# TuringLang/AdvancedVI.jl

Measured on AMD Instinct MI355X. Metric: ELBO-grad-estimates/sec, higher is better.
Workload: dtype f32

## Files before the change

advancedvi.jl_amd/csrc/fr_planes.h:

```cpp
#pragma once
#include "device_common.h"

namespace mivi {

typedef float f32x16 __attribute__((ext_vector_type(16)));
typedef float f32x4 __attribute__((ext_vector_type(4)));
typedef _Float16 f16x8 __attribute__((ext_vector_type(8)));
typedef _Float16 f16x2 __attribute__((ext_vector_type(2)));
typedef unsigned u32x4v __attribute__((ext_vector_type(4)));

constexpr int kFrag = 512;
constexpr int kSplitProducts = 3;
constexpr float kEpsScale = 2048.f;
constexpr float kEpsInv = 1.f / 2048.f;

#define FB_GLDS16(gptr, lptr, off)                                                                         \
  __builtin_amdgcn_global_load_lds((const __attribute__((address_space(1))) void *)(gptr),                 \
                                   (__attribute__((address_space(3))) void *)(lptr), 16, off, 0)

template <int N>
__device__ __forceinline__ void fb_wait_vm() {
  __builtin_amdgcn_s_waitcnt((N & 15) | (7 << 4) | (15 << 8) | ((N >> 4) << 14));
  asm volatile("" ::: "memory");
}
__device__ __forceinline__ void fb_barrier() {
  __builtin_amdgcn_s_waitcnt(0xc07f);
  asm volatile("s_barrier" ::: "memory");
}

__device__ __forceinline__ void fb_scale_of(float amax, float &s, float &inv) {
  unsigned eb = (__builtin_bit_cast(unsigned, amax) >> 23) & 0xffu;
  eb = eb < 25u ? 25u : (eb > 254u ? 254u : eb);
  s = __builtin_bit_cast(float, (267u - eb) << 23);
  inv = __builtin_bit_cast(float, (eb - 13u) << 23);
}

__device__ __forceinline__ void fb_split2(const float *x, u32x4v &uh, u32x4v &ul) {
#pragma unroll
  for (int p = 0; p < 4; ++p) {
    const float a = x[2 * p], b = x[2 * p + 1];
    const _Float16 ah = (_Float16)a, bh = (_Float16)b;
    const float ra = a - (float)ah, rb = b - (float)bh;
    const f16x2 hh = {ah, bh}, ll = {(_Float16)ra, (_Float16)rb};
    uh[p] = __builtin_bit_cast(unsigned, hh);
    ul[p] = __builtin_bit_cast(unsigned, ll);
  }
}
__device__ __forceinline__ float fb_unsplit2(const u32x4v &uh, const u32x4v &ul, int e) {
  const unsigned wh = uh[e >> 1], wl = ul[e >> 1];
  const f16x2 hh = __builtin_bit_cast(f16x2, wh), ll = __builtin_bit_cast(f16x2, wl);
  return (float)hh[e & 1] + (float)ll[e & 1];
}
__device__ __forceinline__ float fb_unsplit2_word(unsigned wh, unsigned wl, int odd) {
  const f16x2 hh = __builtin_bit_cast(f16x2, wh), ll = __builtin_bit_cast(f16x2, wl);
  return (float)hh[odd] + (float)ll[odd];
}
__device__ __forceinline__ void fb_store_frag(unsigned *dst, const float *x) {
  u32x4v uh, ul;
  fb_split2(x, uh, ul);
  store16_wt(dst, uh);
  store16_wt(dst + 256, ul);
}

constexpr int kStageW = 16 * 256;

template <int WJ>
struct FbFrags {
  u32x4v A[2][2], B[WJ][2];
};
__device__ __forceinline__ f32x16 fb_mma(const u32x4v &a, const u32x4v &b, const f32x16 &c) {
  return __builtin_amdgcn_mfma_f32_32x32x16_f16(__builtin_bit_cast(f16x8, a), __builtin_bit_cast(f16x8, b), c, 0, 0, 0);
}
template <int WJ>
__device__ __forceinline__ void fb_group(const FbFrags<WJ> &F, f32x16 (&acc)[2][WJ]) {
  constexpr int PA[3] = {1, 0, 0}, PB[3] = {0, 1, 0};
#pragma unroll
  for (int p = 0; p < 3; ++p)
#pragma unroll
    for (int i = 0; i < 2; ++i)
#pragma unroll
      for (int j = 0; j < WJ; ++j) acc[i][j] = fb_mma(F.A[i][PA[p]], F.B[j][PB[p]], acc[i][j]);
}

template <int OFF>
__device__ __forceinline__ void fb_group_read_asm(f32x16 &acc0, f32x16 &acc1, const FbFrags<1> &Fc, FbFrags<1> &Fn, unsigned ab, unsigned bb) {
  static_assert(OFF >= 0 && OFF + 3072 < 65536, "ds_read_b128 offset field");
  asm volatile(
      "v_mfma_f32_32x32x16_f16 %[c0], %[a0l], %[bh], %[c0]\n\t"
      "ds_read_b128 %[n0h], %[ab] offset:%[o0]\n\t"
      "ds_read_b128 %[n0l], %[ab] offset:%[o1]\n\t"
      "v_mfma_f32_32x32x16_f16 %[c1], %[a1l], %[bh], %[c1]\n\t"
      "ds_read_b128 %[n1h], %[ab] offset:%[o2]\n\t"
      "ds_read_b128 %[n1l], %[ab] offset:%[o3]\n\t"
      "v_mfma_f32_32x32x16_f16 %[c0], %[a0h], %[bl], %[c0]\n\t"
      "ds_read_b128 %[nbh], %[bb] offset:%[o0]\n\t"
      "v_mfma_f32_32x32x16_f16 %[c1], %[a1h], %[bl], %[c1]\n\t"
      "ds_read_b128 %[nbl], %[bb] offset:%[o1]\n\t"
      "v_mfma_f32_32x32x16_f16 %[c0], %[a0h], %[bh], %[c0]\n\t"
      "v_mfma_f32_32x32x16_f16 %[c1], %[a1h], %[bh], %[c1]\n\t"
      "s_waitcnt lgkmcnt(0)"
      : [c0] "+v"(acc0), [c1] "+v"(acc1), [n0h] "=&v"(Fn.A[0][0]), [n0l] "=&v"(Fn.A[0][1]), [n1h] "=&v"(Fn.A[1][0]), [n1l] "=&v"(Fn.A[1][1]),
        [nbh] "=&v"(Fn.B[0][0]), [nbl] "=&v"(Fn.B[0][1])
      : [a0h] "v"(Fc.A[0][0]), [a0l] "v"(Fc.A[0][1]), [a1h] "v"(Fc.A[1][0]), [a1l] "v"(Fc.A[1][1]), [bh] "v"(Fc.B[0][0]), [bl] "v"(Fc.B[0][1]),
        [ab] "v"(ab), [bb] "v"(bb), [o0] "n"(OFF), [o1] "n"(OFF + 1024), [o2] "n"(OFF + 2048), [o3] "n"(OFF + 3072)
      : "memory");
}

template <int WJ>
__device__ __forceinline__ void fb_read_frags(const unsigned *lds, int slot, int wm, int wn, int lane, FbFrags<WJ> &F) {
  const unsigned *cur = lds + slot * kStageW + 4 * lane;
#pragma unroll
  for (int i = 0; i < 2; ++i)
#pragma unroll
    for (int p = 0; p < 2; ++p) F.A[i][p] = *(const u32x4v *)(cur + ((2 * wm + i) * 2 + p) * 256);
#pragma unroll
  for (int j = 0; j < WJ; ++j)
#pragma unroll
    for (int p = 0; p < 2; ++p) F.B[j][p] = *(const u32x4v *)(cur + (8 + (WJ * wn + j) * 2 + p) * 256);
}

}
```

advancedvi.jl_amd/csrc/kernels_fullrank_batch.hip:

```cpp
#include <algorithm>
#include <cstdlib>
#include <type_traits>
#include <cstdio>
#include <vector>

#include "device_common.h"
#include "fr_elem.h"
#include "fr_planes.h"

#ifndef FB_VK
#define FB_VK 0
#endif
#ifndef FB_WJ
#define FB_WJ 1
#endif

namespace mivi {

struct FbArgs {
  int d, M, L;
  int dT, MT;
  const float *params;
  const float *t_mean, *t_istd;
  unsigned *CA;
// ... 295 lines not shown
      FB_GLDS16(sp[f], dst, 0);
      FB_GLDS16(sp[f], dst, 1024);
      sp[f] += gd < gmax[f] ? kFrag : 0;
    }
    ++gd;
  };
  f32x16 acc[2][WJ];
#pragma unroll
  for (int i = 0; i < 2; ++i)
#pragma unroll
    for (int j = 0; j < WJ; ++j)
#pragma unroll
      for (int r = 0; r < 16; ++r) acc[i][j][r] = 0.f;
  const int r32[2] = {R0 + 2 * wm, R0 + 2 * wm + 1};
  const int Gw = (kDG || kSU) ? G : 2 * r32[1] + 2;
  auto after_group = [&](auto S, int g) {
    if constexpr (kDG && (decltype(S)::value & 3) == 3) {
      if (((g + 1) & 7) == 0) {
#pragma unroll
        for (int j = 0; j < WJ; ++j) {
          const float f = tab[((g >> 3) << 7) + 32 * (WJ * wn + j) + l31];
#pragma unroll
          for (int i = 0; i < 2; ++i) {
#pragma unroll
            for (int r = 0; r < 16; ++r) acc[i][j][r] *= f;
          }
        }
        asm volatile("" ::: "memory");
      }
    }
  };
  auto compute = [&](auto S, int g, const FbFrags<WJ> &F) {
    if (!FB_KNOCKED(a, 2)) fb_group<WJ>(F, acc);
    fb_sched_interleave<WJ>();
    after_group(S, g);
  };
  const unsigned lds0 = (unsigned)(uintptr_t)lds + 16u * lane;
  const unsigned ab_lo = lds0 + (2 * wm) * 2 * 1024, bb_lo = lds0 + (8 + WJ * wn * 2) * 1024;
  const unsigned ab_hi = ab_lo + 4 * kStageW * 4, bb_hi = bb_lo + 4 * kStageW * 4;
  (void)ab_hi; (void)bb_hi;
  auto step = [&](auto S, auto VM, auto ISS, int g, const FbFrags<WJ> &Fc, FbFrags<WJ> &Fn) {
    constexpr int sl = decltype(S)::value;
    fb_wait_vm<kPW * decltype(VM)::value>();
    if (!FB_KNOCKED(a, 8)) fb_barrier();
#ifdef MIVI_SB
    __builtin_amdgcn_sched_barrier(0);
#endif
    auto group_and_read = [&]() {
#ifndef MIVI_DEV
      if constexpr (WJ == 1) {
        constexpr int nx = (sl + 1) % NRP, off = (nx & 3) * kStageW * 4;
        fb_group_read_asm<off>(acc[0][0], acc[1][0], Fc, Fn, nx < 4 ? ab_lo : ab_hi, nx < 4 ? bb_lo : bb_hi);
        if constexpr (kDG && (sl & 3) == 3) {
          if (((g + 1) & 7) == 0) asm volatile("s_nop 15\n\ts_nop 7" : "+v"(acc[0][0]), "+v"(acc[1][0])::"memory");
        }
        after_group(S, g);
      } else
#endif
      {
        if (!FB_KNOCKED(a, 4)) fb_read_frags<WJ>(lds, (sl + 1) % NRP, wm, wn, lane, Fn);
        compute(S, g, Fc);
      }
    };
    if constexpr (decltype(ISS)::value) {
      if (!FB_KNOCKED(a, 1)) issue(sl);
      group_and_read();
    } else if (g < Gw) {
      group_and_read();
    }
  };
  FB_STAMP(a, 0);
  FB_NOTE(a, 4, G);
  load_tables();
  static_for<0, NRP>([&](auto S) { issue(decltype(S)::value); });
  fb_wait_vm<kPW * NRP>();
  stage_tables();
  fb_wait_vm<kPW * (NRP - 1)>();
  fb_barrier();
  FB_STAMP(a, 1);
  {
    FbFrags<WJ> F0, F1;
    fb_read_frags<WJ>(lds, 0, wm, wn, lane, F0);
    int g = 0;
    for (; g + NRP < G; g += NRP) {
      static_for<0, NRP>([&](auto S) {
        constexpr int sv = decltype(S)::value;
        if constexpr (sv % 2 == 0) step(S, std::integral_constant<int, NRP - 2>{}, FbT{}, g + sv, F0, F1);
        else step(S, std::integral_constant<int, NRP - 2>{}, FbT{}, g + sv, F1, F0);
      });
    }
    static_for<0, NRP - 1>([&](auto S) {
      constexpr int sv = decltype(S)::value;
      if constexpr (sv % 2 == 0) step(S, std::integral_constant<int, NRP - 2 - sv>{}, FbN{}, g + sv, F0, F1);
      else step(S, std::integral_constant<int, NRP - 2 - sv>{}, FbN{}, g + sv, F1, F0);
    });
    __builtin_amdgcn_s_waitcnt(0xc07f);
    if (g + NRP - 1 < Gw) compute(std::integral_constant<int, NRP - 1>{}, g + NRP - 1, F1);
  }
  f32x16 (&tot)[2][WJ] = acc;
  fb_barrier();
  FB_STAMP(a, 2);
  float *img = reinterpret_cast<float *>(lds) + w * (2 * WJ * kImgW);
  unsigned *WVl = a.WV + (size_t)ln * a.plane_stride;
  unsigned *RPl = a.RP + (size_t)ln * a.plane_stride;
  double *ellp = a.ell_part + (size_t)ln * a.ell_stride;
  const int ncb = a.M >> 5, nmg = a.M >> 4;
  const int ei4 = 4 * (lane & 7);
  float amax[2][4];
  float cmax[WJ][4];
#pragma unroll
  for (int i = 0; i < 2; ++i)
#pragma unroll
    for (int c = 0; c < 4; ++c) amax[i][c] = 0.f;
#pragma unroll
  for (int j = 0; j < WJ; ++j)
#pragma unroll
    for (int p = 0; p < 4; ++p) cmax[j][p] = 0.f;
#pragma unroll
  for (int i = 0; i < 2; ++i) {
    const int lr = 64 * wm + 32 * i;
    f32x4 mu = {0.f, 0.f, 0.f, 0.f}, tm = mu, tis = mu;
    const f32x4 zf = *(const f32x4 *)(vec + 384 + lr + ei4);
    if constexpr (!kDG && !kSU) {
      mu = *(const f32x4 *)(vec + lr + ei4);
      tm = *(const f32x4 *)(vec + 128 + lr + ei4);
      if constexpr (MODE == FB_DIAG) tis = *(const f32x4 *)(vec + 256 + lr + ei4);
    }
#pragma unroll
    for (int j = 0; j < WJ; ++j) {
      float *I = img + (i * WJ + j) * kImgW;
      const int cb32 = (col0 >> 5) + WJ * wn + j;
      const bool pad = 32 * r32[i] >= a.dT || 32 * cb32 >= a.MT;
#pragma unroll
      for (int q = 0; q < 4; ++q) {
        const f32x4 v = {tot[i][j][4 * q], tot[i][j][4 * q + 1], tot[i][j][4 * q + 2], tot[i][j][4 * q + 3]};
        *(f32x4 *)(I + l31 * LDC + 8 * q + 4 * h) = v;
      }
      if constexpr (kSU) {
        const float uf = vec[384 + lr + l31];
        const float wo = a.winv[(size_t)ln * (size_t)(a.M >> 7) * d + (size_t)cb * d + row0 + lr + l31];
#pragma unroll
        for (int g2 = 0; g2 < 2; ++g2) {
          const unsigned *src = WVl + ((size_t)r32[i] * nmg + 2 * cb32 + g2) * kFrag + 4 * lane;
          const u32x4v wh = *(const u32x4v *)src, wl = *(const u32x4v *)(src + 256);
#pragma unroll
          for (int e = 0; e < 8; ++e) {
            float *p = I + (16 * g2 + 8 * (e >> 2) + 4 * h + (e & 3)) * LDC + l31;
            const float x = __builtin_fmaf(*p, uf, fb_unsplit2(wh, wl, e) * wo);
            *p = x;
            amax[i][0] = fmaxf(amax[i][0], fabsf(x));
          }
        }
        continue;
      }
      double s = 0.0;
#pragma unroll
      for (int p = 0; p < 4; ++p) {
        const int en = 8 * p + (lane >> 3);
        const f32x4 v = *(const f32x4 *)(I + en * LDC + ei4) * zf;
        float ell = 0.f;
        f32x4 wv;
        if constexpr (MODE == FB_DIAG) {
          const f32x4 z = mu + v;
#pragma unroll
          for (int c = 0; c < 4; ++c) wv[c] = diag_target_elem(z[c], tm[c], tis[c], ell);
        } else if constexpr (kDR) {
          const f32x4 z = mu + v;
          wv = z - tm;
        } else {
          const unsigned *fr = RPl + ((size_t)cb32 * ng + 2 * r32[i] + (ei4 >> 4)) * kFrag + 4 * (en + 32 * ((ei4 >> 2) & 1)) + 2 * ((ei4 >> 3) & 1);
          const uint2 qh = *(const uint2 *)fr, ql = *(const uint2 *)(fr + 256);
          const float rs = rsv[32 * (WJ * wn + j) + en];
          const unsigned uh[2] = {qh.x, qh.y}, ul[2] = {ql.x, ql.y};
#pragma unroll
          for (int c = 0; c < 4; ++c) wv[c] = dense_target_elem(v[c], fb_unsplit2_word(uh[c >> 1], ul[c >> 1], c & 1) * rs, ell);
        }
        if (pad) { wv = f32x4{0.f, 0.f, 0.f, 0.f}; ell = 0.f; }
        *(f32x4 *)(I + en * LDC + ei4) = wv;
        if constexpr (kDR) {
          cmax[j][p] = fmaxf(cmax[j][p], fmaxf(fmaxf(fabsf(wv[0]), fabsf(wv[1])), fmaxf(fabsf(wv[2]), fabsf(wv[3]))));
        } else {
#pragma unroll
          for (int c = 0; c < 4; ++c) amax[i][c] = fmaxf(amax[i][c], fabsf(wv[c]));
          const double sv = (double)wave_sum_f32(ell);
          s = p ? s + sv : sv;
        }
      }
      if constexpr (!kDR) {
        if (lane == 0) ellp[(size_t)r32[i] * ncb + cb32] = s;
      }
    }
  }
  if constexpr (kDR) {
#pragma unroll
    for (int j = 0; j < WJ; ++j)
#pragma unroll
      for (int p = 0; p < 4; ++p) {
        const float m = fb_lane_max<7>(cmax[j][p]);
        if ((lane & 7) == 0) red[w * 64 + 32 * j + 8 * p + (lane >> 3)] = m;
      }
  } else if constexpr (kSU) {
#pragma unroll
    for (int i = 0; i < 2; ++i) {
      const float m = fb_lane_max<32>(amax[i][0]);
      if (lane < 32) red[w * 64 + 32 * i + lane] = m;
    }
  } else {
#pragma unroll
    for (int i = 0; i < 2; ++i)
#pragma unroll
      for (int c = 0; c < 4; ++c) {
        const float m = fb_lane_max<56>(amax[i][c]);
        if (lane < 8) red[w * 64 + 32 * i + ei4 + c] = m;
      }
  }
  fb_barrier();
  if constexpr (kDR) {
#pragma unroll
    for (int j = 0; j < WJ; ++j) {
      const int cb32 = (col0 >> 5) + WJ * wn + j;
      float s, inv;
      fb_scale_of(fmaxf(red[wn * 64 + 32 * j + l31], red[(NWN + wn) * 64 + 32 * j + l31]), s, inv);
      if (wm == 0 && lane < 32) a.rinv[(size_t)ln * (size_t)(d >> 7) * a.M + (size_t)rb * a.M + col0 + 32 * (WJ * wn + j) + lane] = inv;
#pragma unroll
      for (int i = 0; i < 2; ++i) {
        const float *I = img + (i * WJ + j) * kImgW;
#pragma unroll
        for (int g2 = 0; g2 < 2; ++g2) {
          const f32x4 x0 = *(const f32x4 *)(I + l31 * LDC + 16 * g2 + 4 * h) * s, x1 = *(const f32x4 *)(I + l31 * LDC + 16 * g2 + 8 + 4 * h) * s;
          const float x[8] = {x0[0], x0[1], x0[2], x0[3], x1[0], x1[1], x1[2], x1[3]};
          fb_store_frag(RPl + ((size_t)cb32 * ng + 2 * r32[i] + g2) * kFrag + 4 * lane, x);
        }
      }
    }
  } else {
#pragma unroll
    for (int i = 0; i < 2; ++i) {
      float mx = red[(wm * NWN) * 64 + 32 * i + l31];
#pragma unroll
      for (int x = 1; x < NWN; ++x) mx = fmaxf(mx, red[(wm * NWN + x) * 64 + 32 * i + l31]);
      float s, inv;
      fb_scale_of(mx, s, inv);
      if (wn == 0 && lane < 32) a.winv[(size_t)ln * (size_t)(a.M >> 7) * d + (size_t)cb * d + row0 + 64 * wm + 32 * i + lane] = inv;
#pragma unroll
      for (int j = 0; j < WJ; ++j) {
        const float *I = img + (i * WJ + j) * kImgW;
        const int cb32 = (col0 >> 5) + WJ * wn + j;
#pragma unroll
        for (int g2 = 0; g2 < 2; ++g2) {
          float x[8];
#pragma unroll
          for (int e = 0; e < 8; ++e) x[e] = I[(16 * g2 + 8 * (e >> 2) + 4 * h + (e & 3)) * LDC + l31] * s;
          fb_store_frag(WVl + ((size_t)r32[i] * nmg + 2 * cb32 + g2) * kFrag + 4 * lane, x);
        }
      }
    }
  }
  FB_STAMP(a, 3);
  if (!kDG && !kSU && (flags & 1) && wn == 0 && lane < 32) {
    const int nrb = d >> 5;
#pragma unroll
    for (int i = 0; i < 2; ++i) {
      const int r = 32 * r32[i] + lane;
      float lg, bad;
      logdet_block32(r < a.dT ? a.params[a.dT + (size_t)r * a.dT + r] : 1.f, lg, bad);
      if (lane == 0) {
        a.ld_part[r32[i]] = (double)lg;
        a.ld_part[nrb + r32[i]] = (double)bad;
      }
    }
  }
}

__device__ __forceinline__ void fb_value_block(const FbArgs &a, int l, double *red) {
  const int d = a.d;
  ValueIn vin{};
  vin.ell_const = a.ell_const;
  vin.ell_part = a.ell_part + (size_t)l * a.ell_stride;
  vin.n_ell_part = (d >> 5) * (a.M >> 5);
  vin.he_part = a.he_part + (size_t)l * a.he_stride;
  vin.n_he_part = (d >> 6) * (a.M >> 5);
  vin.ld_part = a.ld_part;
  vin.n_ld_part = d >> 5;
  OutArgs out{};
  const bool last = l == a.lane_last && a.value_last;
  out.value = last ? a.value_last : a.values + (size_t)l * a.value_stride;
  if (a.parts) {
    out.partials_mode = 1;
    out.partials = a.parts + (size_t)l * a.part_stride;
    out.scalars_off = (int64_t)d + (int64_t)(d >> 7) * ((d >> 7) + 1) / 2 * 16384;
  }
  out.ent_kind = a.ent_kind;
  out.M_total = a.M_total;
  out.M_local = a.MT;
  out.status = a.status;
  const float *pp = a.params;
  const int dT = a.dT;
  finalize_value_block<float, 256, false>(dT, vin, out, (int64_t)dT + (int64_t)dT * dT, [pp, dT](int i) { return pp[dT + (size_t)i * dT + i]; }, red);
}

template <int WJ, int NRV, int TABW, int WPE, bool PART = false>
__global__ __launch_bounds__(512 / WJ, WPE / WJ) void k_fb_vjp(FbArgs a) {
  static_assert(WJ == 1, "the transposing B reads are written for the 64 x 32 wave tiles");
  constexpr int LDC = 36, NF = WJ, kPW = 2 * WJ;
  constexpr int NR = NRV;
  constexpr int kBody = (NR * kStageW > 16 * kImgW / 2) ? NR * kStageW : 16 * kImgW / 2;
  __shared__ __attribute__((aligned(16))) unsigned lds[kBody + TABW];
  float *wf = reinterpret_cast<float *>(lds + kBody);
  const int tid = threadIdx.x, lane = tid & 63, l31 = lane & 31, h = lane >> 5;
  const int w = __builtin_amdgcn_readfirstlane(tid >> 6);
  const int wm = w / (4 / WJ), wn = w % (4 / WJ);
  if ((int)blockIdx.x < a.L) {
    if (tid < 256) fb_value_block(a, (int)blockIdx.x, reinterpret_cast<double *>(lds));
    return;
  }
  const __attribute__((address_space(4))) int *wp = (const __attribute__((address_space(4))) int *)a.work + 4 * ((int)blockIdx.x - a.L);
  const int ln = wp[0], rc = wp[1];
  const int rb = rc & 0xffff, cb = rc >> 16;
  const int d = a.d, M = a.M, nmg = M >> 4, dT = a.dT;
  const int row0 = rb * 128, col0 = cb * 128;
  const bool last = ln == a.lane_last && a.grad_last;
  float *grad = last ? a.grad_last : a.grads + (size_t)ln * a.grad_stride;
  const bool upper = a.write_upper || last;
  const int G = nmg;
  const int NB = M >> 7;
  const unsigned *sp[NF];
  unsigned btr;
  {
    const int G4 = lane >> 4, c16 = lane & 15;
    const int kgpar = G4 & 1, hq = G4 >> 1, hp = c16 & 1, half = (c16 >> 1) & 1, sl = 4 * hq + (c16 >> 2);
    btr = 16u * (unsigned)(8 * (2 * hp + kgpar) + ((sl & 7) ^ (4 * hp))) + 8u * (unsigned)half;
  }
#pragma unroll
  for (int f = 0; f < NF; ++f) {
    const int fs = NF * w + f, fr = fs & 3;
    if (fs < 4) {
      sp[f] = a.WV + (size_t)ln * a.plane_stride + ((size_t)((row0 >> 5) + fr) * nmg) * kFrag + 4 * lane;
    } else {
      const int m8 = lane >> 3, s8 = m8 >> 2, hp = (m8 >> 1) & 1, kgpar = m8 & 1, sl = 8 * s8 + ((lane & 7) ^ (4 * hp));
      sp[f] = a.epsP + (size_t)ln * a.plane_stride + ((size_t)((col0 >> 4) + 2 * fr + kgpar)) * kFrag + 4 * (sl + 32 * hp);
    }
  }
  int gi = 0;
  const int bstep_odd = (d >> 4) * kFrag - 64;
  constexpr int kMaxNBv = 16;
  float twi[kMaxNBv];
  auto load_table = [&]() {
    if (tid < 128) {
      const float *wi = a.winv + (size_t)ln * (size_t)NB * d + row0 + tid;
#pragma unroll
      for (int r = 0; r < kMaxNBv; ++r) twi[r] = wi[(size_t)(r < NB ? r : NB - 1) * d];
    }
    asm volatile("" ::: "memory");
  };
  auto build_table = [&]() {
    if (tid < 128) {
      float u = twi[0], grow = 1.f;
#pragma unroll
      for (int r = 1; r < kMaxNBv; ++r) {
        if (r < NB) {
          float ratio = u / twi[r];
          if (!(ratio <= 1099511627776.f)) ratio = 1099511627776.f;
          if (ratio > 1.f && grow * ratio > 1.2089258e24f) ratio = fmaxf(1.2089258e24f / grow, 1.f);
          if (ratio > 1.f) grow *= ratio;
          wf[(r - 1) * 128 + tid] = ratio;
          u = u / ratio;
        }
      }
      wf[(NB - 1) * 128 + tid] = u;
    }
  };
  auto issue = [&](int slot) {
#pragma unroll
    for (int f = 0; f < NF; ++f) {
      unsigned *dst = lds + slot * kStageW + (NF * w + f) * 512;
      if (!(FB_VK & 16)) {
        FB_GLDS16(sp[f], dst, 0);
        FB_GLDS16(sp[f], dst, 1024);
      }
      if (NF * w + f >= 4) sp[f] += (gi & 1) ? bstep_odd : 64;
      else sp[f] += kFrag;
    }
    ++gi;
  };
  auto read_frags = [&](int slot, FbFrags<WJ> &F) {
    if ((FB_VK & 64)) return;
    const unsigned *cur = lds + slot * kStageW + 4 * lane;
#pragma unroll
    for (int i = 0; i < 2; ++i)
#pragma unroll
      for (int p = 0; p < 2; ++p) F.A[i][p] = *(const u32x4v *)(cur + ((2 * wm + i) * 2 + p) * 256);
    const unsigned bb = (unsigned)(uintptr_t)(lds + slot * kStageW) + (8 + 2 * wn) * 1024 + btr;
    uint2 t0, t1, t2, t3;
    asm volatile("ds_read_b64_tr_b16 %0, %4\n\tds_read_b64_tr_b16 %1, %4 offset:512\n\tds_read_b64_tr_b16 %2, %4 offset:1024\n\t"
                 "ds_read_b64_tr_b16 %3, %4 offset:1536\n\ts_waitcnt lgkmcnt(0)"
                 : "=&v"(t0), "=&v"(t1), "=&v"(t2), "=&v"(t3) : "v"(bb) : "memory");
    F.B[0][0] = u32x4v{t0.x, t0.y, t1.x, t1.y};
    F.B[0][1] = u32x4v{t2.x, t2.y, t3.x, t3.y};
  };
  const int ri[2] = {(row0 >> 5) + 2 * wm, (row0 >> 5) + 2 * wm + 1};
  int cj[WJ];
#pragma unroll
  for (int j = 0; j < WJ; ++j) cj[j] = (col0 >> 5) + WJ * wn + j;
  const bool work = cj[0] <= ri[1];
  bool dg[2];
#pragma unroll
  for (int i = 0; i < 2; ++i) {
    dg[i] = false;
#pragma unroll
    for (int j = 0; j < WJ; ++j) dg[i] = dg[i] || ri[i] == cj[j];
  }
  f32x16 acc[2][WJ];
#pragma unroll
  for (int i = 0; i < 2; ++i)
#pragma unroll
    for (int j = 0; j < WJ; ++j)
#pragma unroll
      for (int r = 0; r < 16; ++r) acc[i][j][r] = 0.f;
  double rsd[2] = {0.0, 0.0};
  float rcur[2] = {0.f, 0.f};
  auto after_group = [&](auto S, int g, const FbFrags<WJ> &F) {
    if (__builtin_expect(dg[0] || dg[1], 0)) {
#pragma unroll
      for (int i = 0; i < 2; ++i)
        if (dg[i]) {
#pragma unroll
          for (int e = 0; e < 8; ++e) rcur[i] += fb_unsplit2(F.A[i][0], F.A[i][1], e);
        }
    }
    if constexpr (decltype(S)::value == 3 || decltype(S)::value == -1) {
      if (((g + 1) & 7) == 0 && g + 1 < G) {
        const float *wr = wf + ((g >> 3) << 7) + 64 * wm;
#pragma unroll
        for (int i = 0; i < 2; ++i) {
#pragma unroll
          for (int q = 0; q < 4; ++q) {
            const f32x4 f4 = *(const f32x4 *)(wr + 32 * i + 8 * q + 4 * h);
#pragma unroll
            for (int j = 0; j < WJ; ++j)
#pragma unroll
              for (int c = 0; c < 4; ++c) acc[i][j][4 * q + c] *= f4[c];
          }
          rsd[i] = (rsd[i] + (double)rcur[i]) * (double)wr[32 * i + l31];
          rcur[i] = 0.f;
        }
        asm volatile("" ::: "memory");
      }
    }
  };
  auto compute = [&](auto S, int g, const FbFrags<WJ> &F) {
    if (!(FB_VK & 32)) fb_group<WJ>(F, acc);
    after_group(S, g, F);
  };
  {
    FB_STAMP(a, 0);
    FB_NOTE(a, 4, G);
    load_table();
#pragma unroll
    for (int s0 = 0; s0 < NR - 1; ++s0) issue(s0);
    fb_wait_vm<kPW * (NR - 1)>();
    build_table();
    int slot = 0;
    for (int g = 0; g < G; ++g) {
      if (g == 1) FB_STAMP(a, 1);
      if (g + NR - 2 < G) fb_wait_vm<kPW * (NR - 2)>();
      else if (NR > 3 && g + 1 < G) fb_wait_vm<kPW>();
      else fb_wait_vm<0>();
      fb_barrier();
      if (g + NR - 1 < G) issue(slot == 0 ? NR - 1 : slot - 1);
      if (work) {
        FbFrags<WJ> F;
        read_frags(slot, F);
        compute(std::integral_constant<int, -1>{}, g, F);
      }
      slot = slot == NR - 1 ? 0 : slot + 1;
    }
  }
  fb_barrier();
  FB_STAMP(a, 2);
  if ((FB_VK & 128)) return;
  float *Cs = reinterpret_cast<float *>(lds) + w * kImgW;
  const float *wfin = wf + (NB - 1) * 128 + 64 * wm;
  const double invM = 1.0 / (double)a.M_total;
  const bool pow2M = (a.M_total & (a.M_total - 1)) == 0;
  const float invMe = (float)invM * kEpsInv;
  const double direct = direct_entropy_coeff(a.ent_kind);
  const int i4 = 4 * (lane & 7);
#pragma unroll
  for (int i = 0; i < 2; ++i) {
#pragma unroll
    for (int j = 0; j < WJ; ++j) {
      if (cj[j] > ri[i] || 32 * ri[i] >= dT) continue;
      const bool diag = ri[i] == cj[j];
      const int rbase = 32 * ri[i], cbase = 32 * cj[j];
#pragma unroll
      for (int q = 0; q < 4; ++q) {
        const f32x4 v = {acc[i][j][4 * q], acc[i][j][4 * q + 1], acc[i][j][4 * q + 2], acc[i][j][4 * q + 3]};
        *(f32x4 *)(Cs + l31 * LDC + 8 * q + 4 * h) = v;
      }
      const f32x4 ff = *(const f32x4 *)(wfin + 32 * i + i4);
#pragma unroll
      for (int p = 0; p < 4; ++p) {
        const int n = 8 * p + (lane >> 3);
        const int gi = rbase + i4, gj = cbase + n;
        float cjj = 1.f;
        if (diag && gj >= gi && gj < gi + 4) cjj = a.params[dT + (size_t)gj * dT + gj];
        const f32x4 v = *(const f32x4 *)(Cs + n * LDC + i4) * ff;
        f32x4 o;
        if constexpr (PART) {
          o = v * kEpsInv;
          if (diag) {
#pragma unroll
            for (int c = 0; c < 4; ++c) o[c] = gj > gi + c ? 0.f : o[c];
          }
          store16_wt(a.parts + (size_t)ln * a.part_stride + d + ((size_t)(rb * (rb + 1) / 2 + cb) << 14) + (size_t)(gj - col0) * 128 + (gi - row0), o);
          continue;
        }
        if (!diag && pow2M) {
          o = -v * invMe;
        } else {
#pragma unroll
          for (int c = 0; c < 4; ++c) o[c] = vjp_elem(v[c] * kEpsInv, gi + c, gj, pow2M, (float)invM, invM, direct, cjj);
        }
        store16_wt(grad + dT + (size_t)gj * dT + gi, o);
      }
      if (!PART && !diag && upper) {
        const f32x4 z4 = {0.f, 0.f, 0.f, 0.f};
#pragma unroll
        for (int p = 0; p < 4; ++p) {
          const int ii = 8 * p + (lane >> 3);
          store16_wt(grad + dT + (size_t)(rbase + ii) * dT + cbase + i4, z4);
        }
      }
      asm volatile("s_waitcnt lgkmcnt(0)" ::: "memory");
    }
    if (dg[i] && 32 * ri[i] < dT) {
      const double mine = (rsd[i] + (double)rcur[i]) * (double)wfin[32 * i + l31];
      const double sm = mine + __shfl_xor(mine, 32, 64);
      if constexpr (PART) {
        if (lane < 32) a.parts[(size_t)ln * a.part_stride + 32 * ri[i] + lane] = (float)sm;
      } else {
        if (lane < 32) grad[32 * ri[i] + lane] = dmu_elem(sm, invM);
      }
    }
  }
  FB_STAMP(a, 3);
}

__global__ __launch_bounds__(256) void k_fb_finalize_parts(FbArgs a) {
  __shared__ double red[4 * 4];
  const int d = a.d, l = blockIdx.y, j = blockIdx.x, tid = threadIdx.x;
  const float *P = a.parts + (size_t)l * a.part_stride;
  const bool last = l == a.lane_last && a.grad_last;
  float *grad = last ? a.grad_last : a.grads + (size_t)l * a.grad_stride;
  const bool upper = a.write_upper || last;
  const double invM = 1.0 / (double)a.M_total;
  const bool pow2M = (a.M_total & (a.M_total - 1)) == 0;
  const double direct = direct_entropy_coeff(a.ent_kind);
  if (j == d) {
    for (int i = tid; i < d; i += 256) grad[i] = dmu_elem((double)P[i], invM);
    double s_ld = 0.0, bad = 0.0;
    for (int i = tid; i < d; i += 256) {
      const double c = (double)a.params[d + (size_t)i * d + i];
      if (!(c > 0.0)) bad = 1.0;
      s_ld += log(c);
    }
    double v[2] = {s_ld, bad};
    block_sum_n<double, 256, 2>(v, red);
    if (tid == 0) {
      const int64_t so = (int64_t)d + (int64_t)(d >> 7) * ((d >> 7) + 1) / 2 * 16384;
      const double sum_ell = (double)P[so], s_he = (double)P[so + 1], Mt = (double)a.M_total;
      const double ent = (ent_is_closed(a.ent_kind) ? 0.5 * d * (1.0 + kLog2Pi) : s_he / Mt + 0.5 * d * kLog2Pi) + v[0];
      const double value = -(sum_ell / Mt + ent);
      float *vo = (l == a.lane_last && a.value_last) ? a.value_last : a.values + (size_t)l * a.value_stride;
      *vo = (float)value;
      int st = 0;
      if (!isfinite(value)) st |= 1;
      if (v[1] > 0.0) st |= 2;
      if (st && a.status) atomicOr(a.status, st);
    }
    return;
  }
  const int cb = j >> 7, lj = j & 127;
  const float cjj = a.params[d + (size_t)j * d + j];
  for (int i4 = 4 * tid; i4 < d; i4 += 1024) {
    f32x4 o = {0.f, 0.f, 0.f, 0.f};
    if (i4 + 3 >= j) {
      const int rb = i4 >> 7;
      const f32x4 v = *(const f32x4 *)(P + d + ((size_t)(rb * (rb + 1) / 2 + cb) << 14) + (size_t)lj * 128 + (i4 & 127));
#pragma unroll
      for (int c = 0; c < 4; ++c) o[c] = vjp_elem(v[c], i4 + c, j, pow2M, (float)invM, invM, direct, cjj);
    } else if (!upper) {
      continue;
    }
    *(f32x4 *)(grad + d + (size_t)j * d + i4) = o;
  }
}

namespace {
constexpr int kBM = 128, kBN = 128;
constexpr int kWJ = FB_WJ;
constexpr int kOwnCuTilesPerCU10 = 17;

void fb_upload(DevBuf &b, const void *src, size_t bytes) {
  if (b.bytes < bytes || !b.p) {
    if (b.p) (void)hipFree(b.p);
    (void)hipMalloc(&b.p, bytes);
    b.bytes = bytes;
  }
  (void)hipMemcpy(b.p, src, bytes, hipMemcpyHostToDevice);
}
}

static int fb_pad(int x) { return (x + 127) / 128 * 128; }
bool fb_shape_ok(const mivi_ctx *c, int M) {
  static const bool off = getenv("MIVI_BATCH_GEN3") && atoi(getenv("MIVI_BATCH_GEN3")) == 0;
  return !off && c->cfg.family == MIVI_FULLRANK && c->cfg.dtype == MIVI_F32 && c->cfg.d % 32 == 0 && M % 32 == 0 && c->cfg.d >= kBM &&
         c->cfg.d <= 2048 && M >= 128 && M <= 2048;
}
bool fb_whole_tiles(const mivi_ctx *c, int M) { return c->cfg.d % kBM == 0 && M % kBN == 0; }
size_t fb_plane_words(const mivi_ctx *c, int M) { return (size_t)fb_pad(c->cfg.d) * fb_pad(M) / 512 * kFrag; }
size_t fb_cplane_words(const mivi_ctx *c) { return (size_t)(fb_pad(c->cfg.d) / 32) * (fb_pad(c->cfg.d) / 16) * kFrag; }
size_t fb_part_len(const mivi_ctx *c) {
  const size_t d = (size_t)c->cfg.d, T = d / 128;
  return (d + T * (T + 1) / 2 * 16384 + 2 + 3) / 4 * 4;
}

const FbTab *fb_prepare(mivi_ctx *c, int M, int L) {
  FbTables &ft = c->fb;
  for (FbTab &t : ft.tab)
    if (t.L == L && t.M == M && t.prod.p && t.vjp.p) return &t;
  FbTab &t = ft.tab[ft.next_tab];
  ft.next_tab = (ft.next_tab + 1) & 3;
  invalidate_graph(c);
  (void)hipStreamSynchronize(c->stream);
  t.L = t.M = 0;
  const int d = fb_pad(c->cfg.d), nrb = d / kBM, ncb = fb_pad(M) / kBN;
  std::vector<std::vector<int4>> lists(8);
  int panel = 0;
  for (int l = 0; l < L; ++l)
    for (int cb = 0; cb < ncb; ++cb, ++panel)
      for (int rb = nrb - 1; rb >= 0; --rb) lists[panel % 8].push_back(make_int4(l, rb | (cb << 16), (l == 0 && cb == 0) ? 1 : 0, 0));
  while (true) {
    int a = 0, b = 0;
    for (int x = 1; x < 8; ++x) {
      if (lists[x].size() > lists[a].size()) a = x;
      if (lists[x].size() < lists[b].size()) b = x;
    }
    if (lists[a].size() <= lists[b].size() + 1) break;
    lists[b].push_back(lists[a].back());
    lists[a].pop_back();
  }
  for (auto &li : lists) std::stable_sort(li.begin(), li.end(), [](const int4 &p, const int4 &q) { return (p.y & 0xffff) > (q.y & 0xffff); });
  std::vector<int4> prod;
  size_t mx = 0;
  for (auto &li : lists) mx = std::max(mx, li.size());
  for (size_t i = 0; i < mx; ++i)
    for (int x = 0; x < 8; ++x)
      if (i < lists[x].size()) prod.push_back(lists[x][i]);
  std::vector<int4> flat;
  for (int l = 0; l < L; ++l)
    for (int rb = 0; rb < nrb; ++rb)
      for (int cb = 0; cb <= rb; ++cb) flat.push_back(make_int4(l, rb | (cb << 16), 0, 0));
  std::vector<int4> vjp;
  {
    const size_t n = flat.size();
    size_t pos = 0;
    std::vector<std::vector<int4>> lx(8);
    for (int x = 0; x < 8; ++x) {
      const size_t e = (n * (x + 1)) / 8;
      for (; pos < e; ++pos) lx[x].push_back(flat[pos]);
    }
    size_t m2 = 0;
    for (auto &li : lx) m2 = std::max(m2, li.size());
    for (size_t i = 0; i < m2; ++i)
      for (int x = 0; x < 8; ++x)
        if (i < lx[x].size()) vjp.push_back(lx[x][i]);
  }
  std::vector<int4> prod2;
  const size_t panel_bytes = (size_t)kBM * d * 4;
  constexpr int NG = 4, NC = 8 / NG;
  if (nrb % NG == 0 && (size_t)(nrb / NG) * panel_bytes <= (1u << 20)) {
    std::vector<std::vector<int4>> lp(8);
    int pn = 0;
    for (int l = 0; l < L; ++l)
      for (int cb = 0; cb < ncb; ++cb, ++pn)
        for (int rg = 0; rg < NG; ++rg)
          for (int r = 0; r < nrb / NG; ++r) lp[rg + NG * (pn % NC)].push_back(make_int4(l, (rg * (nrb / NG) + r) | (cb << 16), 0, 0));
    size_t m3 = 0;
    for (auto &li : lp) m3 = std::max(m3, li.size());
    for (size_t i = 0; i < m3; ++i)
      for (int x = 0; x < 8; ++x)
        if (i < lp[x].size()) prod2.push_back(lp[x][i]);
  } else {
    for (int l = 0; l < L; ++l)
      for (int cb = 0; cb < ncb; ++cb)
        for (int rb = 0; rb < nrb; ++rb) prod2.push_back(make_int4(l, rb | (cb << 16), 0, 0));
  }
  std::vector<int4> prod3;
  for (auto &li : lists) std::stable_sort(li.begin(), li.end(), [](const int4 &p, const int4 &q) { return (p.y & 0xffff) < (q.y & 0xffff); });
  for (size_t i = 0; i < mx; ++i)
    for (int x = 0; x < 8; ++x)
      if (i < lists[x].size()) prod3.push_back(lists[x][i]);
  fb_upload(t.prod, prod.data(), prod.size() * sizeof(int4));
  fb_upload(t.vjp, vjp.data(), vjp.size() * sizeof(int4));
  fb_upload(t.prod2, prod2.data(), prod2.size() * sizeof(int4));
  fb_upload(t.prod3, prod3.data(), prod3.size() * sizeof(int4));
  if (!t.prod.p || !t.vjp.p || !t.prod2.p || !t.prod3.p) return nullptr;
  t.n_prod2 = (int)prod2.size();
  t.n_prod = (int)prod.size();
  t.n_vjp = (int)vjp.size();
  t.L = L;
  t.M = M;
  return &t;
}

static FbArgs fb_args(mivi_ctx *c, const void *params, int M_true) {
  FbTables &t = c->fb;
  const int d = fb_pad(c->cfg.d), M = fb_pad(M_true);
  FbArgs a{};
  a.d = d; a.M = M;
  a.dT = c->cfg.d; a.MT = M_true;
  a.params = (const float *)params;
  a.t_mean = (const float *)c->t_mean.p;
  a.t_istd = (const float *)c->t_istd.p;
  a.CA = (unsigned *)t.CA.p;
  a.cscale = (float *)t.cscale.p;
  a.pscale = (float *)t.pscale.p;
  a.tscale = (float *)t.tscale.p;
  a.winv = (float *)t.winv.p;
  a.rinv = (float *)t.rinv.p;
  a.epsP = (unsigned *)t.epsP.p;
  a.WV = (unsigned *)t.WV.p;
  a.t_prec = (const float *)c->t_prec.p; a.dP = c->dP;
  a.PA = (unsigned *)t.PA.p;
  a.RP = (unsigned *)t.RP.p;
  a.Tinv = (const float *)t.Tinv.p;
  a.TA = (unsigned *)t.TA.p;
  a.plane_stride = (long long)fb_plane_words(c, M);
  a.ell_part = (double *)t.ell.p; a.ell_stride = (long long)(d / 32) * (M / 32);
  a.he_part = (double *)t.he.p; a.he_stride = (long long)(d / 64) * (M / 32);
  a.ld_part = (double *)t.ld.p;
  a.ent_kind = c->cfg.entropy; a.M_total = c->M_total;
  a.status = (int *)c->status.p;
  a.ell_const = c->t_const;
  return a;
}

void fb_launch_eps(mivi_ctx *c, const FbStep &s, bool with_cplanes, hipStream_t stream) {
  const int d = fb_pad(c->cfg.d), M = fb_pad(s.M), L = s.L;
  FbArgs a = fb_args(c, s.params, s.M);
  a.L = L;
  a.rng = s.rng;
  a.obj = s.obj;
  const int gx = (d / 64) * (M / 32) / 2;
  a.n_riders = with_cplanes ? (4 * (d / 32) + gx - 1) / gx : 0;
  hipLaunchKernelGGL(k_fb_eps, dim3(gx, L + a.n_riders), dim3(512), 0, stream, a);
}
void fb_launch_pplanes(mivi_ctx *c, hipStream_t stream) {
  FbArgs a = fb_args(c, nullptr, c->cfg.n_mc);
  hipLaunchKernelGGL(k_fb_pplanes, dim3(c->cfg.d / 32, 4), dim3(512), 0, stream, a);
}
void fb_launch_tplanes(mivi_ctx *c, hipStream_t stream) {
  FbArgs a = fb_args(c, nullptr, c->cfg.n_mc);
  hipLaunchKernelGGL(k_fb_tplanes, dim3(c->cfg.d / 32, 4), dim3(512), 0, stream, a);
}
void fb_launch_compute(mivi_ctx *c, const FbStep &s, hipStream_t stream, int which) {
  const FbTab &tb = *s.tab;
  FbArgs a = fb_args(c, s.params, s.M);
  a.L = s.L;
  a.grads = (float *)s.grads; a.grad_stride = s.grad_stride;
  a.values = (float *)s.values; a.value_stride = s.value_stride;
  a.grad_last = (float *)s.grad_last; a.value_last = (float *)s.value_last; a.lane_last = s.lane_last;
  a.write_upper = s.write_upper;
  a.parts = (float *)s.parts; a.part_stride = s.part_stride;
  if (s.obj) { a.ent_kind = s.ent_kind; a.M_total = s.M; }
#ifdef MIVI_DEV
  static long long *dbg_buf = nullptr;
  static const bool dbg_on = getenv("MIVI_FB_DBG") != nullptr;
  if (dbg_on && !dbg_buf) (void)hipMalloc(&dbg_buf, 2 * 8192 * 8 * sizeof(long long));
  auto dump = [&](const char *name, int n) {
    if (!dbg_on) return;
    (void)hipStreamSynchronize(stream);
    std::vector<long long> h((size_t)n * 8);
    (void)hipMemcpy(h.data(), dbg_buf, h.size() * 8, hipMemcpyDeviceToHost);
    long long t0 = h[0], t3 = 0;
    for (int i = 0; i < n; ++i) { t0 = std::min(t0, h[(size_t)i * 8]); t3 = std::max(t3, h[(size_t)i * 8 + 3]); }
    double pro = 0, loop = 0, epi = 0, pg = 0; long long gs = 0;
    for (int i = 0; i < n; ++i) { const long long *r = &h[(size_t)i * 8]; pro += r[1] - r[0]; loop += r[2] - r[1]; epi += r[3] - r[2]; gs += r[4]; }
    pg = loop / (double)gs;
    fprintf(stderr, "[fbdbg] %s: %d workgroups, span %.2f us | mean prologue %.2f us, main loop %.2f us (%.3f us per group), epilogue %.2f us | last start %.2f us\n", name, n, (t3 - t0) * 0.01, pro / n * 0.01, loop / n * 0.01, pg * 0.01, epi / n * 0.01, 0.0);
    std::vector<long long> st; for (int i = 0; i < n; ++i) st.push_back(h[(size_t)i * 8] - t0);
    std::sort(st.begin(), st.end());
    fprintf(stderr, "[fbdbg]   starts (us): p25 %.2f p50 %.2f p75 %.2f p90 %.2f max %.2f\n", st[n / 4] * 0.01, st[n / 2] * 0.01, st[3 * n / 4] * 0.01, st[9 * n / 10] * 0.01, st[n - 1] * 0.01);
  };
  a.dbg = dbg_on ? dbg_buf : nullptr;
  a.knock = getenv("MIVI_FB_KNOCK") ? atoi(getenv("MIVI_FB_KNOCK")) : 0;
#endif
  a.work = (const int4 *)tb.prod.p; a.n_work = tb.n_prod;
  const int n_cu = c->n_cu > 0 ? c->n_cu : 256;
  auto own_cu_for = [&](int n, bool equal_tiles) {
#ifdef MIVI_DEV
    static const int force_ring = getenv("MIVI_FB_RING") ? atoi(getenv("MIVI_FB_RING")) : 0;
    if (force_ring == 4) return false;
    if (force_ring == 8) return true;
#endif
    const int gmax = fb_pad(c->cfg.d) / 16;
    const int thr10 = gmax <= 32 ? 10 : (gmax <= 64 ? 10 + (gmax - 32) * 7 / 32 : kOwnCuTilesPerCU10 + (gmax - 64 < 64 ? gmax - 64 : 64) * 5 / 64);
    return !equal_tiles && n > n_cu && 10 * (long long)n <= (long long)thr10 * n_cu;
  };
  auto prod = [&](auto MODE, int n) {
    constexpr int md = decltype(MODE)::value;
    if (own_cu_for(n, md == FB_DENSE_G)) hipLaunchKernelGGL((k_fb_prod<kWJ, md, 8>), dim3(n), dim3(512 / kWJ), 0, stream, a);
    else hipLaunchKernelGGL((k_fb_prod<kWJ, md, 4>), dim3(n), dim3(512 / kWJ), 0, stream, a);
  };
  if (s.dense) {
    if (which & 1) prod(std::integral_constant<int, FB_DENSE_R>{}, tb.n_prod);
    a.work = (const int4 *)tb.prod2.p; a.n_work = tb.n_prod2;
    if (which & 4) prod(std::integral_constant<int, FB_DENSE_G>{}, tb.n_prod2);
  } else if (which & 1) {
    prod(std::integral_constant<int, FB_DIAG>{}, tb.n_prod);
#ifdef MIVI_DEV
    dump("k_fb_prod<DIAG>", tb.n_prod);
#endif
  }
  if (s.stl && (which & 8)) {
    a.work = (const int4 *)tb.prod3.p; a.n_work = tb.n_prod;
    prod(std::integral_constant<int, FB_STL_U>{}, tb.n_prod);
  }
  a.work = (const int4 *)tb.vjp.p; a.n_work = tb.n_vjp;
  if (s.values_only) {
    if (which & 2) hipLaunchKernelGGL((k_fb_vjp<kWJ, 3, 256, 6>), dim3(s.L), dim3(512 / kWJ), 0, stream, a);
    return;
  }
  if (which & 2) {
    if (s.parts) {
      if (a.M <= 256) hipLaunchKernelGGL((k_fb_vjp<kWJ, 3, 256, 6, true>), dim3(tb.n_vjp + s.L), dim3(512 / kWJ), 0, stream, a);
// ... 23 lines not shown
```

Measured before the change: 352,800.

## Swap MFMA operand order to produce transposed accumulators and drop LDS transpose epilogue

The MFMA operands are swapped so each accumulator holds the transposed tile: lane index maps to the row and register index to the column. This lets the per-row scale become a single scalar multiply per lane instead of per-register vector loads. The epilogue writes gradients straight from registers with 4-byte stores, dropping the LDS staging buffer, its barrier and the lgkmcnt wait. LDS shrinks to the pipeline stages only, which may raise occupancy. In exchange, 16-byte stores become strided 4-byte stores; lanes still write contiguous addresses across a row, so the stores stay coalesced.

```diff
diff --git a/advancedvi.jl_amd/csrc/fr_planes.h b/advancedvi.jl_amd/csrc/fr_planes.h
--- a/advancedvi.jl_amd/csrc/fr_planes.h
+++ b/advancedvi.jl_amd/csrc/fr_planes.h
@@ -81,6 +81,16 @@
 #pragma unroll
       for (int j = 0; j < WJ; ++j) acc[i][j] = fb_mma(F.A[i][PA[p]], F.B[j][PB[p]], acc[i][j]);
 }
+template <int WJ>
+__device__ __forceinline__ void fb_group_swapped(const FbFrags<WJ> &F, f32x16 (&acc)[2][WJ]) {
+  constexpr int PA[3] = {1, 0, 0}, PB[3] = {0, 1, 0};
+#pragma unroll
+  for (int p = 0; p < 3; ++p)
+#pragma unroll
+    for (int i = 0; i < 2; ++i)
+#pragma unroll
+      for (int j = 0; j < WJ; ++j) acc[i][j] = fb_mma(F.B[j][PB[p]], F.A[i][PA[p]], acc[i][j]);
+}
 
 template <int OFF>
 __device__ __forceinline__ void fb_group_read_asm(f32x16 &acc0, f32x16 &acc1, const FbFrags<1> &Fc, FbFrags<1> &Fn, unsigned ab, unsigned bb) {
diff --git a/advancedvi.jl_amd/csrc/kernels_fullrank_batch.hip b/advancedvi.jl_amd/csrc/kernels_fullrank_batch.hip
--- a/advancedvi.jl_amd/csrc/kernels_fullrank_batch.hip
+++ b/advancedvi.jl_amd/csrc/kernels_fullrank_batch.hip
@@ -621,9 +621,9 @@
 template <int WJ, int NRV, int TABW, int WPE, bool PART = false>
 __global__ __launch_bounds__(512 / WJ, WPE / WJ) void k_fb_vjp(FbArgs a) {
   static_assert(WJ == 1, "the transposing B reads are written for the 64 x 32 wave tiles");
-  constexpr int LDC = 36, NF = WJ, kPW = 2 * WJ;
+  constexpr int NF = WJ, kPW = 2 * WJ;
   constexpr int NR = NRV;
-  constexpr int kBody = (NR * kStageW > 16 * kImgW / 2) ? NR * kStageW : 16 * kImgW / 2;
+  constexpr int kBody = NR * kStageW;
   __shared__ __attribute__((aligned(16))) unsigned lds[kBody + TABW];
   float *wf = reinterpret_cast<float *>(lds + kBody);
   const int tid = threadIdx.x, lane = tid & 63, l31 = lane & 31, h = lane >> 5;
@@ -752,15 +752,10 @@
         const float *wr = wf + ((g >> 3) << 7) + 64 * wm;
 #pragma unroll
         for (int i = 0; i < 2; ++i) {
-#pragma unroll
-          for (int q = 0; q < 4; ++q) {
-            const f32x4 f4 = *(const f32x4 *)(wr + 32 * i + 8 * q + 4 * h);
-#pragma unroll
-            for (int j = 0; j < WJ; ++j)
-#pragma unroll
-              for (int c = 0; c < 4; ++c) acc[i][j][4 * q + c] *= f4[c];
-          }
-          rsd[i] = (rsd[i] + (double)rcur[i]) * (double)wr[32 * i + l31];
+          const float fr = wr[32 * i + l31];
+#pragma unroll
+          for (int j = 0; j < WJ; ++j) acc[i][j] *= fr;
+          rsd[i] = (rsd[i] + (double)rcur[i]) * (double)fr;
           rcur[i] = 0.f;
         }
         asm volatile("" ::: "memory");
@@ -768,7 +763,7 @@
     }
   };
   auto compute = [&](auto S, int g, const FbFrags<WJ> &F) {
-    if (!(FB_VK & 32)) fb_group<WJ>(F, acc);
+    if (!(FB_VK & 32)) fb_group_swapped<WJ>(F, acc);
     after_group(S, g, F);
   };
   {
@@ -795,10 +790,8 @@
       slot = slot == NR - 1 ? 0 : slot + 1;
     }
   }
-  fb_barrier();
   FB_STAMP(a, 2);
   if ((FB_VK & 128)) return;
-  float *Cs = reinterpret_cast<float *>(lds) + w * kImgW;
   const float *wfin = wf + (NB - 1) * 128 + 64 * wm;
   const double invM = 1.0 / (double)a.M_total;
   const bool pow2M = (a.M_total & (a.M_total - 1)) == 0;
@@ -812,36 +805,36 @@
       if (cj[j] > ri[i] || 32 * ri[i] >= dT) continue;
       const bool diag = ri[i] == cj[j];
       const int rbase = 32 * ri[i], cbase = 32 * cj[j];
+      const int gi = rbase + l31;
+      const float ff = wfin[32 * i + l31];
+      float cii = 1.f;
+      if (diag) cii = a.params[dT + (size_t)gi * dT + gi];
+      float *dst;
+      size_t ldo;
+      if constexpr (PART) {
+        dst = a.parts + (size_t)ln * a.part_stride + d + ((size_t)(rb * (rb + 1) / 2 + cb) << 14) + (size_t)(cbase + 4 * h - col0) * 128 + (gi - row0);
+        ldo = 128;
+      } else {
+        dst = grad + dT + (size_t)(cbase + 4 * h) * dT + gi;
+        ldo = (size_t)dT;
+      }
 #pragma unroll
       for (int q = 0; q < 4; ++q) {
-        const f32x4 v = {acc[i][j][4 * q], acc[i][j][4 * q + 1], acc[i][j][4 * q + 2], acc[i][j][4 * q + 3]};
-        *(f32x4 *)(Cs + l31 * LDC + 8 * q + 4 * h) = v;
-      }
-      const f32x4 ff = *(const f32x4 *)(wfin + 32 * i + i4);
-#pragma unroll
-      for (int p = 0; p < 4; ++p) {
-        const int n = 8 * p + (lane >> 3);
-        const int gi = rbase + i4, gj = cbase + n;
-        float cjj = 1.f;
-        if (diag && gj >= gi && gj < gi + 4) cjj = a.params[dT + (size_t)gj * dT + gj];
-        const f32x4 v = *(const f32x4 *)(Cs + n * LDC + i4) * ff;
-        f32x4 o;
-        if constexpr (PART) {
-          o = v * kEpsInv;
-          if (diag) {
-#pragma unroll
-            for (int c = 0; c < 4; ++c) o[c] = gj > gi + c ? 0.f : o[c];
+#pragma unroll
+        for (int c = 0; c < 4; ++c) {
+          const int gj = cbase + 8 * q + 4 * h + c;
+          const float v = acc[i][j][4 * q + c] * ff;
+          float o;
+          if constexpr (PART) {
+            o = v * kEpsInv;
+            if (diag) o = gj > gi ? 0.f : o;
+          } else if (!diag && pow2M) {
+            o = -v * invMe;
+          } else {
+            o = vjp_elem(v * kEpsInv, gi, gj, pow2M, (float)invM, invM, direct, cii);
           }
-          store16_wt(a.parts + (size_t)ln * a.part_stride + d + ((size_t)(rb * (rb + 1) / 2 + cb) << 14) + (size_t)(gj - col0) * 128 + (gi - row0), o);
-          continue;
-        }
-        if (!diag && pow2M) {
-          o = -v * invMe;
-        } else {
-#pragma unroll
-          for (int c = 0; c < 4; ++c) o[c] = vjp_elem(v[c] * kEpsInv, gi + c, gj, pow2M, (float)invM, invM, direct, cjj);
-        }
-        store16_wt(grad + dT + (size_t)gj * dT + gi, o);
+          store4_wt(dst + (size_t)(8 * q + c) * ldo, o);
+        }
       }
       if (!PART && !diag && upper) {
         const f32x4 z4 = {0.f, 0.f, 0.f, 0.f};
@@ -851,7 +844,6 @@
           store16_wt(grad + dT + (size_t)(rbase + ii) * dT + cbase + i4, z4);
         }
       }
-      asm volatile("s_waitcnt lgkmcnt(0)" ::: "memory");
     }
     if (dg[i] && 32 * ri[i] < dT) {
       const double mine = (rsd[i] + (double)rcur[i]) * (double)wfin[32 * i + l31];
```

Result: no change. 355,900, median of 5 (+0.9%).
